# ssheybani/baby-vision-curriculum

Hardware: AMD Instinct MI355X
Metric: video clips/sec (node) VideoMAE-base 16x224^2 bf16 pretraining (higher is better)
Workload: dtype bf16; 1 GPU; VideoMAE-base (ViT-B/16 encoder, 4-layer decoder), 16x224x224 clips, tubelet 2, 90% tube mask, full training step (fwd + MSE + bwd + GradScaler + SGD-Nesterov); clips_per_gpu=256, global_batch=256, parallelism=dp1, weights=random init N(0,0.02), seed 0

## Files before the change

baby-vision-curriculum_amd/csrc/gemm8.hip:

```cpp
#include <stdio.h>
#include <stdlib.h>

#include <type_traits>

#include "gemm_tile.h"
#include "rowops.h"

namespace bvc {

namespace {

typedef __attribute__((ext_vector_type(4))) unsigned int u32x4;

#ifndef BVC_G8_ST_AUX
#define BVC_G8_ST_AUX 0
#endif
#ifndef BVC_G8_ROW_ST_AUX
#define BVC_G8_ROW_ST_AUX 0
#endif
constexpr uint32_t kInvalidBase = 0x80000000u;

struct Unit {
    int pi, m0, n0, kt0, nkt, split, tile;
};

__device__ __forceinline__ bf16x8 tr_frag(uint32_t region, uint32_t lane_base, uint32_t lane_swz, uint32_t chunk16, int ks) {
    const uint32_t a = region + lane_base + (chunk16 ^ lane_swz) + (uint32_t)ks * 8192u;
    bf16x4 lo = __builtin_amdgcn_ds_read_tr16_b64_v4i16((AS3 bf16x4*)(size_t)a);
    bf16x4 hi = __builtin_amdgcn_ds_read_tr16_b64_v4i16((AS3 bf16x4*)(size_t)(a + 1024u));
    return __builtin_shufflevector(lo, hi, 0, 1, 2, 3, 4, 5, 6, 7);
}

__device__ __forceinline__ float row16_sum(float v) {
    v += __builtin_bit_cast(float, __builtin_amdgcn_update_dpp(0, __builtin_bit_cast(int, v), 0x128, 0xF, 0xF, false));
    v += __builtin_bit_cast(float, __builtin_amdgcn_update_dpp(0, __builtin_bit_cast(int, v), 0x124, 0xF, 0xF, false));
    v += __builtin_bit_cast(float, __builtin_amdgcn_update_dpp(0, __builtin_bit_cast(int, v), 0x122, 0xF, 0xF, false));
    v += __builtin_bit_cast(float, __builtin_amdgcn_update_dpp(0, __builtin_bit_cast(int, v), 0x121, 0xF, 0xF, false));
    return v;
}

template <int BM, int BN>
__device__ __forceinline__ void decode_unit(const GemmGroup& g, int uid, Unit& u) {
    const bool tail = g.bal_units > 0 && uid >= g.bal_units;
    const int S = tail ? g.prob[0].split_k : 1;
    const int key = tail ? (uid - g.bal_units) * S : uid;
    int pi = 0;
#pragma unroll
    for (int i = 1; i < kMaxGroup; ++i)
        if (i < g.nprob && key >= g.tile_start[i]) pi = i;
    const GemmProblem& p = g.prob[pi];
    const int lid = tail ? (key - g.tile_start[pi]) / S : uid - g.tile_start[pi];
    const int tiles_n = (p.N + BN - 1) / BN, tiles_m = (p.M + BM - 1) / BM;
    const int ntiles = tiles_m * tiles_n;
    const int G = g.panel[pi];
    int split, tm, tn;
    if (tail) {
        split = S;
        tm = lid / tiles_n; tn = lid - tm * tiles_n;
    } else if (G > 0) {
        split = lid / ntiles;
        tile_of(lid - split * ntiles, tiles_m, tiles_n, G, tm, tn);
    } else if (G == -1) {
        split = lid / ntiles;
        const int w = lid - split * ntiles;
        if (tiles_n > tiles_m) { tm = w % tiles_m; tn = w / tiles_m; } else { tm = w / tiles_n; tn = w % tiles_n; }
    } else {
        split = lid % p.split_k;
        const int tl = lid / p.split_k;
        const bool m_fast = tiles_n > tiles_m;
        tm = m_fast ? tl % tiles_m : tl / tiles_n;
        tn = m_fast ? tl / tiles_m : tl % tiles_n;
    }
    const int nt_all = (p.K + 63) / 64;
    int per = (nt_all + p.split_k - 1) / p.split_k;
    per = (per + 1) & ~1;
    int kt0 = split * per;
    if (g.bal_units > 0) {
        kt0 = split * g.bal_lb;
        per = tail ? (nt_all - kt0 + 1) & ~1 : g.bal_lb;
    }
    u.pi = pi;
    u.m0 = __builtin_amdgcn_readfirstlane(tm * BM);
    u.n0 = __builtin_amdgcn_readfirstlane(tn * BN);
    u.kt0 = __builtin_amdgcn_readfirstlane(kt0);
    u.nkt = __builtin_amdgcn_readfirstlane(per);
    u.split = __builtin_amdgcn_readfirstlane(split);
    u.tile = __builtin_amdgcn_readfirstlane(tm * tiles_n + tn);
}

}

template <int BM, int BN, bool AT, bool BT, int EC>
__global__ __launch_bounds__(512, 1) void gemm8_kernel(const GemmGroup g, const int total_units) {
    extern __shared__ __attribute__((aligned(16))) char smem[];
    static_assert(BM == 256 || (BM == 128 && BN == 384), "128-row tiles: the 128 x 384 geometry only");
    static_assert(BN == 256 || BN == 128 || (BN == 384 && BM == 128), "column tiles of 256 / 128, or 384 with 128 rows");
    static_assert((EC == 4 || EC == 5) == (BM == 128 && !AT), "row epilogues (EC 4 / 5) are the k-contiguous-A instantiations of the 128 x 384 tile, and only they");
    static_assert(BM == 256 || EC == 4 || EC == 5 || (AT && BT && (EC == 2 || EC == 6)), "128 x 384 with transposed A: weight gradients");
    static_assert(EC != 6 || (AT && BT), "EC 6 (deterministic weight gradients) is a TN product");
    static_assert(EC != 4 || !BT, "EC 4 (residual + LayerNorm forward) is an NT product");
    constexpr int A_BYTES = BM * 64 * 2, B_BYTES = BN * 64 * 2, TILE = A_BYTES + B_BYTES;
    constexpr int WMR = BM / 2;
    constexpr int WN = BN / 4, TN = WN / 16, TM = WMR / 16, TMH = TM / 2;
    constexpr int NB = BN / 64, NBH = BN / 128, NAH = BM / 128;
    constexpr int n0c = AT ? NBH : (NB == 6 ? 3 : NB < 2 ? NB : 2), n1c = AT ? NAH : NB - n0c, n2c = AT ? NBH : BM / 128, n3c = AT ? NAH : BM / 128;
    constexpr int RT = BM / 128;
    constexpr int KMAX = (n0c > 2 || n1c > 2 || n2c > 2 || n3c > 2) ? 3 : 2;
    constexpr int PT = n0c + n1c + n2c + n3c;
#ifdef BVC_G8_DMA_LATE
    constexpr bool LATE = true;
#else
    constexpr bool LATE = false;
#endif
    constexpr int PAR_BYTES = EC == 4 ? 3 * BN * 4 : EC == 5 ? BN * 4 : 0, STAT_OFF = PAR_BYTES, COL_OFF = STAT_OFF + 4096;
    constexpr int CPR = BN == 384 ? 8 : WN / 8;
    constexpr int NSIDE = TM * (16 / (64 / CPR));
    static_assert(PT + 2 * NSIDE < 64, "vmcnt is a 6-bit counter");
    constexpr int WP = AT ? PT : n3c + n0c + n1c;
    constexpr int W1 = LATE ? n0c + n1c + n2c : PT;
    constexpr int W3 = LATE ? (AT ? n2c + n3c + n0c : n3c + n0c) : WP;

    const int tid = threadIdx.x, lane = tid & 63;
    const int wave = __builtin_amdgcn_readfirstlane(tid >> 6);
    const int wm = wave >> 2, wn = wave & 3;

    const int xcd = blockIdx.x & 7, slot_id = blockIdx.x >> 3, nslots = gridDim.x >> 3;
    const int xq = total_units >> 3, xr = total_units & 7;
    const int x_lo = xcd < xr ? xcd * (xq + 1) : xr * (xq + 1) + (xcd - xr) * xq;
    const int x_hi = x_lo + xq + (xcd < xr ? 1 : 0);
    int uid = x_lo + slot_id, u_step = nslots, u_hi = x_hi;
    if (EC == 2 && g.bal_units > 0) {
        u_step = 1;
        if (uid < x_hi) {
            u_hi = uid + 1;
        } else {
            const int J = xcd * nslots - x_lo + (uid - x_hi), I = 8 * nslots - g.bal_units;
            uid = g.bal_units + (J * g.bal_tiles) / I;
            u_hi = g.bal_units + ((J + 1) * g.bal_tiles) / I;
        }
    }
    if (uid >= u_hi) {
        if constexpr (EC == 5) {
            float* pr = g.prob[0].ln_part + (size_t)blockIdx.x * 2 * BN;
            for (int i = tid; i < 2 * BN; i += 512) pr[i] = 0.f;
        }
        return;
    }
    if constexpr (EC == 4 || EC == 5) {
        const int cnt = x_hi - x_lo, r = cnt % nslots, nmax = (cnt + nslots - 1) / nslots;
        int num = 0, den = 1;
        if (r > 0 && slot_id >= r) { num = slot_id - r + 1; den = nslots - r + 1; }
        else if (r == 0 && nmax >= 4) { num = slot_id; den = 2 * nslots; }
        const int quanta = __builtin_amdgcn_readfirstlane((int)((long long)g.stagger * num / den));
        for (int i = 0; i < quanta / 127; ++i) __builtin_amdgcn_s_sleep(127);
    }
    if (BVC_DBG(g, 1024) && (slot_id & 1)) {
        for (int i = 0; i < ((g.dbg >> 12) & 63); ++i) __builtin_amdgcn_s_sleep(127);
    }

    Unit su;
    decode_unit<BM, BN>(g, uid, su);
    int s_uid = uid, s_kt = 0;
    bool s_valid = true;
    __amdgpu_buffer_rsrc_t s_ra, s_rb;
    uint32_t s_la, s_lb, s_baseA, s_baseB, s_strideA, s_strideB;
    auto s_problem = [&]() {
        const GemmProblem& p = g.prob[su.pi];
        s_ra = make_rsrc(p.A, p.a_bytes);
        s_rb = make_rsrc(p.B, p.b_bytes);
        if constexpr (!AT) {
            const int r = 8 * wave + (lane >> 3);
            s_la = (uint32_t)((r * p.lda + (((lane & 7) ^ swz_rows(r)) << 3)) * 2);
            s_strideA = (uint32_t)(64 * p.lda * 2);
        } else {
            const int kr = 4 * wave + (lane >> 4);
            s_la = (uint32_t)((kr * p.lda + (((lane & 15) ^ swz_tr<128>(kr)) << 3)) * 2);
            s_strideA = (uint32_t)(32 * p.lda * 2);
        }
        if constexpr (!BT) {
            const int r = 8 * wave + (lane >> 3);
            s_lb = (uint32_t)((r * p.ldb + (((lane & 7) ^ swz_rows(r)) << 3)) * 2);
            s_strideB = (uint32_t)(64 * p.ldb * 2);
        } else {
            const int kr = 4 * wave + (lane >> 4);
            s_lb = (uint32_t)((kr * p.ldb + (((lane & 15) ^ swz_tr<128>(kr)) << 3)) * 2);
            s_strideB = (uint32_t)(32 * p.ldb * 2);
        }
    };
    auto s_ktile = [&]() {
        const GemmProblem& p = g.prob[su.pi];
        const int kt = su.kt0 + s_kt;
        const bool ok = s_valid && kt * 64 < p.K;
        const int k0 = kt * 64;
        s_baseA = !ok ? kInvalidBase : AT ? (uint32_t)((k0 * p.lda + su.m0) * 2) : (uint32_t)((su.m0 * p.lda + k0) * 2);
        s_baseB = !ok ? kInvalidBase : BT ? (uint32_t)((k0 * p.ldb + su.n0) * 2) : (uint32_t)((su.n0 * p.ldb + k0) * 2);
    };
    auto s_advance = [&]() {
        if (++s_kt == su.nkt) {
            s_kt = 0;
            s_uid += u_step;
            if (s_uid < u_hi) {
                const int old = su.pi;
                decode_unit<BM, BN>(g, s_uid, su);
                if (su.pi != old) s_problem();
            } else {
                s_valid = false;
            }
        }
        s_ktile();
    };
    const uint32_t lds_base = (uint32_t)(size_t)((AS3 char*)smem);
    const uint32_t lds0 = lds_base + (uint32_t)wave * 1024u;
    const uint32_t tr_base = (uint32_t)((8 * (lane >> 4) + ((lane >> 2) & 3)) * 256 + ((lane & 3) >> 1) * 16 + (lane & 1) * 8);
    const uint32_t tr_swz = (uint32_t)swz_tr<128>(8 * (lane >> 4) + ((lane >> 2) & 3)) << 4;
    auto b_region = [&](int j) -> uint32_t { return (uint32_t)(A_BYTES + ((wn * WN + 16 * j) >> 7) * 16384); };
    auto b_chunk16 = [&](int j) -> uint32_t { return (uint32_t)(2 * ((wn * WN + 16 * j) & 127)); };
    const uint32_t a_region = BM == 256 ? (uint32_t)wm * 16384u : 0u;
    const uint32_t a_chunk0 = BM == 256 ? 0u : (uint32_t)wm * 128u;
    auto load_a = [&](char* region, int j) {
        const uint32_t off = s_la + s_baseA + (AT ? (uint32_t)(j & 1) * s_strideA + (uint32_t)(j >> 1) * 256u : (uint32_t)j * s_strideA);
        glds16(s_ra, off, lds0 + (uint32_t)(region - smem) + (uint32_t)j * 8192u);
    };
    auto load_b = [&](char* region, int j) {
        const uint32_t off = s_lb + s_baseB + (BT ? (uint32_t)(j & 1) * s_strideB + (uint32_t)(j >> 1) * 256u : (uint32_t)j * s_strideB);
        glds16(s_rb, off, lds0 + (uint32_t)(region - smem) + (uint32_t)j * 8192u);
    };
    using I0 = std::integral_constant<int, 0>;
    using I1 = std::integral_constant<int, 1>;
    using I2 = std::integral_constant<int, 2>;
    using I3 = std::integral_constant<int, 3>;
    auto stage_one = [&](auto gi_, auto k_, char* buf) {
        constexpr int GI = decltype(gi_)::value, K = decltype(k_)::value;
        char* ra_ = buf;
        char* rb_ = buf + A_BYTES;
        if constexpr (!AT) {
            if constexpr (GI == 0) { if constexpr (K < n0c) load_b(rb_, K); }
            else if constexpr (GI == 1) { if constexpr (K < n1c) load_b(rb_, n0c + K); }
            else if constexpr (GI == 2) { if constexpr (K < n2c) load_a(ra_, BM == 256 ? (K == 0 ? 0 : 2) : 0); }
            else { if constexpr (K < n3c) load_a(ra_, BM == 256 ? (K == 0 ? 1 : 3) : 1); }
        } else {
            if constexpr (GI == 0) { if constexpr (K < NBH) load_b(rb_, 2 * K); }
            else if constexpr (GI == 1) { if constexpr (K < NAH) load_a(ra_, 2 * K); }
            else if constexpr (GI == 2) { if constexpr (K < NBH) load_b(rb_, 2 * K + 1); }
            else { if constexpr (K < NAH) load_a(ra_, 2 * K + 1); }
        }
        if constexpr (GI == 3 && K == KMAX - 1) s_advance();
    };
    auto stage_group = [&](auto gi_, char* buf) {
        stage_one(gi_, I0{}, buf); stage_one(gi_, I1{}, buf);
        if constexpr (KMAX == 3) stage_one(gi_, I2{}, buf);
    };
    auto stage_phase = [&](auto q_, auto k_, char* cur, char* oth) {
        constexpr int Q = decltype(q_)::value;
        if constexpr (Q == 0) stage_one(I2{}, k_, oth);
        else if constexpr (Q == 1) stage_one(I3{}, k_, oth);
        else if constexpr (Q == 2) stage_one(I0{}, k_, cur);
        else stage_one(I1{}, k_, cur);
    };

    char* const buf0 = smem;
    char* const buf1 = smem + TILE;
    constexpr int PARK = BN == 384 ? 16 * 48 * 4 : 16 * WN * 4;
    AS3 char* const wl = (AS3 char*)smem + 2 * TILE + wave * PARK;

    if constexpr (EC == 0) {
        const GemmProblem& p0 = g.prob[0];
        AS3 float* lbias = (AS3 float*)((AS3 char*)smem + 2 * TILE);
        const int npad = ((p0.N + BN - 1) / BN) * BN;
        for (int i = tid; i < npad; i += 512) lbias[i] = (p0.bias && i < p0.N) ? p0.bias[i] : 0.f;
        __syncthreads();
    }
    if constexpr (EC == 4 || EC == 5) {
        const GemmProblem& p0 = g.prob[0];
        AS3 float* lpar = (AS3 float*)((AS3 char*)smem + 2 * TILE);
        for (int i = tid; i < BN; i += 512) {
            if constexpr (EC == 4) {
                lpar[i] = p0.bias ? p0.bias[i] : 0.f;
                lpar[BN + i] = p0.ln_gamma[i];
                lpar[2 * BN + i] = p0.ln_beta[i];
            } else {
                lpar[i] = p0.ln_gamma[i];
            }
        }
        if constexpr (EC == 5) {
            AS3 float* lcol = (AS3 float*)((AS3 char*)smem + 2 * TILE + COL_OFF);
            for (int i = tid; i < 8 * 2 * WN; i += 512) lcol[i] = 0.f;
        }
        __syncthreads();
    }
    s_problem();
    s_ktile();
    stage_group(I0{}, buf0); stage_group(I1{}, buf0); stage_group(I2{}, buf0); stage_group(I3{}, buf0);
    stage_group(I0{}, buf1); stage_group(I1{}, buf1);
    wait_vmcnt<WP>();
    asm volatile("s_barrier" ::: "memory");
#ifndef BVC_G8_NO_STAGGER
    if (wm == 1) asm volatile("s_barrier" ::: "memory");
#endif

    Unit cu;
    decode_unit<BM, BN>(g, uid, cu);
    int after_epi = 0;


    while (true) {
        const GemmProblem& p = g.prob[cu.pi];
        f32x4 acc[TM][TN];
#pragma unroll
        for (int i = 0; i < TM; ++i)
#pragma unroll
            for (int j = 0; j < TN; ++j) acc[i][j] = f32x4{0.f, 0.f, 0.f, 0.f};
        float rsum[2] = {0.f, 0.f};
        const bool do_rowsum = (EC == 2 || EC == 6) && p.rowsum != nullptr && cu.n0 == 0;

        auto ktile = [&](auto rs_, char* cur, char* oth) {
            constexpr bool RS = decltype(rs_)::value;
            const char* la = cur;
            const char* lb = cur + A_BYTES;
            if constexpr (!AT) {
                bf16x8 bfr[2][TN];
                auto phase = [&](auto q_) {
                    constexpr int q = decltype(q_)::value;
                    __builtin_amdgcn_sched_barrier(0);
#ifdef BVC_G8_DMA_FIRST
                    if constexpr (!LATE) { stage_phase(q_, I0{}, cur, oth); stage_phase(q_, I1{}, cur, oth); if constexpr (KMAX == 3) stage_phase(q_, I2{}, cur, oth); }
#endif
                    uint32_t sw = tr_swz;
                    if constexpr (BT && q == 0) asm volatile("" : "+v"(sw));
                    if constexpr (q == 0) {
#pragma unroll
                        for (int ks = 0; ks < 2; ++ks)
#pragma unroll
                            for (int j = 0; j < TN; ++j)
                                bfr[ks][j] = BT ? tr_frag(lds_base + (uint32_t)(cur - smem) + b_region(j), tr_base, sw, b_chunk16(j), ks)
                                                : read_frag<BN, false>(lb, wn * WN + 16 * j, ks, lane);
                    }
                    bf16x8 af[2][RT];
#pragma unroll
                    for (int ks = 0; ks < 2; ++ks)
#pragma unroll
                        for (int ii = 0; ii < RT; ++ii)
                            af[ks][ii] = read_frag<256, false>(la, BM == 256 ? wm * WMR + 16 * (2 * q + ii) : 32 * q + 16 * wm, ks, lane);
#ifndef BVC_G8_DMA_FIRST
                    if constexpr (!LATE) { stage_phase(q_, I0{}, cur, oth); stage_phase(q_, I1{}, cur, oth); if constexpr (KMAX == 3) stage_phase(q_, I2{}, cur, oth); }
#endif
                    if constexpr (q == 1) {
                        if (after_epi == 0) wait_vmcnt<W1>();
                        else if (after_epi == NSIDE) wait_vmcnt<W1 + NSIDE>();
                        else if (after_epi == 2 * NSIDE) wait_vmcnt<W1 + 2 * NSIDE>();
                    }
                    if constexpr (q == 3) wait_vmcnt<W3>();
                    asm volatile("s_barrier" ::: "memory");
                    __builtin_amdgcn_sched_barrier(0);
                    __builtin_amdgcn_s_setprio(1);
                    constexpr int NM = 2 * RT * TN;
#pragma unroll
                    for (int t = 0; t < NM; ++t) {
                        const int ks = t / (RT * TN), ii = (t / TN) % RT, j = t % TN;
                        acc[RT * q + ii][j] = __builtin_amdgcn_mfma_f32_16x16x32_bf16(bfr[ks][j], af[ks][ii], acc[RT * q + ii][j], 0, 0, 0);
                        if constexpr (LATE) {
                            if (t == NM / 4 - 1) stage_phase(q_, I0{}, cur, oth);
                            if (t == NM / 2 - 1) stage_phase(q_, I1{}, cur, oth);
                        }
                    }
                    __builtin_amdgcn_s_setprio(0);
                    __builtin_amdgcn_sched_barrier(0);
                    asm volatile("s_barrier" ::: "memory");
                };
                phase(I0{}); phase(I1{}); phase(I2{}); phase(I3{});
            } else {
                bf16x8 bfr[TN];
                auto phase = [&](auto q_) {
                    constexpr int q = decltype(q_)::value;
                    constexpr int ks = q >> 1, mh = q & 1;
                    __builtin_amdgcn_sched_barrier(0);
                    bf16x8 af[TMH];
                    uint32_t sw = tr_swz;
                    asm volatile("" : "+v"(sw));
                    const uint32_t slot = lds_base + (uint32_t)(cur - smem);
                    if constexpr (mh == 0) {
#pragma unroll
                        for (int j = 0; j < TN; ++j) bfr[j] = tr_frag(slot + b_region(j), tr_base, sw, b_chunk16(j), ks);
                    }
#pragma unroll
                    for (int ii = 0; ii < TMH; ++ii) af[ii] = tr_frag(slot + a_region, tr_base, sw, a_chunk0 + 32u * (TMH * mh + ii), ks);
                    if constexpr (!LATE) {
                        stage_phase(q_, I0{}, cur, oth); stage_phase(q_, I1{}, cur, oth);
                        if constexpr (KMAX == 3) stage_phase(q_, I2{}, cur, oth);
                    }
                    if constexpr (q == 1) {
                        if (after_epi == 0) wait_vmcnt<W1>();
                        else if (after_epi == NSIDE) wait_vmcnt<W1 + NSIDE>();
                        else if (after_epi == 2 * NSIDE) wait_vmcnt<W1 + 2 * NSIDE>();
                    }
                    if constexpr (q == 3) wait_vmcnt<W3>();
                    asm volatile("s_barrier" ::: "memory");
                    __builtin_amdgcn_sched_barrier(0);
                    __builtin_amdgcn_s_setprio(1);
                    constexpr int NM = TMH * TN;
#pragma unroll
                    for (int t = 0; t < NM; ++t) {
                        const int ii = t / TN, j = t % TN;
                        acc[TMH * mh + ii][j] = __builtin_amdgcn_mfma_f32_16x16x32_bf16(bfr[j], af[ii], acc[TMH * mh + ii][j], 0, 0, 0);
                        if constexpr (LATE) {
                            if (t == NM / 4 - 1) stage_phase(q_, I0{}, cur, oth);
                            if (t == NM / 2 - 1) stage_phase(q_, I1{}, cur, oth);
                        }
                    }
                    if (RS && do_rowsum && wn < TMH) {
                        bf16x8 a;
                        if constexpr (TMH == 4) {
                            switch (wn) {
                                case 0: a = af[0]; break;
                                case 1: a = af[1]; break;
                                case 2: a = af[2]; break;
                                default: a = af[3]; break;
                            }
                        } else {
                            a = wn == 0 ? af[0] : af[1];
                        }
                        union { bf16x8 v; uint32_t u[4]; } w;
                        w.v = a;
                        float t0 = 0.f, t1 = 0.f;
#pragma unroll
                        for (int e = 0; e < 4; ++e) {
                            t0 += __uint_as_float(w.u[e] << 16);
                            t1 += __uint_as_float(w.u[e] & 0xffff0000u);
                        }
                        rsum[mh] += t0 + t1;
                    }
                    __builtin_amdgcn_s_setprio(0);
                    __builtin_amdgcn_sched_barrier(0);
                    asm volatile("s_barrier" ::: "memory");
                };
                phase(I0{}); phase(I1{}); phase(I2{}); phase(I3{});
            }
            after_epi = 0;
        };

        for (int kt = 0; kt < cu.nkt; kt += 2) {
            ktile(std::bool_constant<EC == 2 || EC == 6>{}, buf0, buf1);
            ktile(std::bool_constant<EC == 2 || EC == 6>{}, buf1, buf0);
        }

        const int m0 = cu.m0, n0 = cu.n0;
        const int epi = p.epi, Mrows = p.M, Ncols = p.N, ldc = p.ldc;
        int seg_shift = 0;
        if constexpr (EC == 4 || EC == 5) {
            if (p.seg_rows > 0) {
                const int upc = p.seg_rows >> 7, u = m0 >> 7, c = u / upc;
                seg_shift = __builtin_amdgcn_readfirstlane(c * p.seg_stride + p.seg_off + ((u - c * upc) << 7) - m0);
            }
        }
        const float alpha = p.alpha_dev ? p.alpha * p.alpha_dev[0] : p.alpha;
        constexpr int UNITS = WN / 4;
        constexpr int RPU = 64 / CPR;
        constexpr int U = 16 / RPU;
        static_assert(NSIDE == TM * U, "epilogue geometry");
        int nstores = 0;
        constexpr uint32_t kDrop = 0xFFFFFFF0u;
        auto park = [&](int i) {
            const int row = lane & 15;
#pragma unroll
            for (int j = 0; j < TN; ++j) {
                const int unit = (4 * j + (lane >> 4)) ^ (row & (UNITS - 1));
                *reinterpret_cast<AS3 f32x4*>(wl + row * (WN * 4) + unit * 16) = acc[i][j];
            }
        };
        const bool atomic = p.split_k > 1 || g.accum != 0;
        if constexpr (EC == 0) {
            const __amdgpu_buffer_rsrc_t rc = make_rsrc(p.C, BVC_DBG(g, 1) ? 0u : kDrop);
            const __amdgpu_buffer_rsrc_t rc2 = make_rsrc(p.C2 ? p.C2 : p.C, BVC_DBG(g, 1) ? 0u : kDrop);
            const AS3 float* lbias = (const AS3 float*)((AS3 char*)smem + 2 * TILE);
            const int q4 = lane >> 4;
            f32x4 bj[TN];
#pragma unroll
            for (int j = 0; j < TN; ++j) {
                const int nb = n0 + wn * WN + 16 * j + 4 * q4;
                bj[j] = *reinterpret_cast<const AS3 f32x4*>(lbias + nb);
            }
            const bool two_out = epi == EPI_GELU;
            const bool relu = epi == EPI_RELU;
            const int ncol = n0 + wn * WN + 16 * (q4 & 1) + 8 * (q4 >> 1);
#pragma unroll
            for (int i = 0; i < TM; ++i) {
                const int m = m0 + wm * WMR + 16 * i + (lane & 15);
#pragma unroll
                for (int jp = 0; jp < TN / 2; ++jp) {
                    float va[4], vb[4];
#pragma unroll
                    for (int e = 0; e < 4; ++e) {
                        va[e] = acc[i][2 * jp][e] * alpha + bj[2 * jp][e];
                        vb[e] = acc[i][2 * jp + 1][e] * alpha + bj[2 * jp + 1][e];
                    }
                    if (relu) {
#pragma unroll
                        for (int e = 0; e < 4; ++e) { va[e] = fmaxf(va[e], 0.f); vb[e] = fmaxf(vb[e], 0.f); }
                    }
                    const int n = ncol + 32 * jp;
                    const uint32_t o = (m < Mrows && n < Ncols) ? (uint32_t)(((size_t)m * ldc + n) * 2) : kDrop;
                    auto emit = [&](__amdgpu_buffer_rsrc_t r) {
                        uint32_t a0 = pack2bf(va[0], va[1]), a1 = pack2bf(va[2], va[3]);
                        uint32_t b0 = pack2bf(vb[0], vb[1]), b1 = pack2bf(vb[2], vb[3]);
                        const auto s0 = __builtin_amdgcn_permlane16_swap(a0, b0, false, false);
                        const auto s1 = __builtin_amdgcn_permlane16_swap(a1, b1, false, false);
                        __builtin_amdgcn_raw_buffer_store_b128(u32x4{s0[0], s1[0], s0[1], s1[1]}, r, o, 0, BVC_G8_ST_AUX);
                    };
                    if (two_out) {
                        float vv[8], gg[8];
#pragma unroll
                        for (int e = 0; e < 4; ++e) { vv[e] = va[e]; vv[4 + e] = vb[e]; }
                        gelu_split(vv, gg);
#pragma unroll
                        for (int e = 0; e < 4; ++e) { va[e] = vv[e]; vb[e] = vv[4 + e]; }
                        emit(rc);
#pragma unroll
                        for (int e = 0; e < 4; ++e) { va[e] = gg[e]; vb[e] = gg[4 + e]; }
                        emit(rc2);
                    } else {
                        emit(rc);
                    }
                }
            }
            nstores = two_out ? 2 * NSIDE : NSIDE;
        } else if constexpr (EC == 4) {
            const uint32_t ext = (uint32_t)Mrows * (uint32_t)(BN * 4);
            const __amdgpu_buffer_rsrc_t rres = make_rsrc(p.resid + (size_t)seg_shift * BN, ext), rc = make_rsrc(p.C, ext), rc2 = make_rsrc(p.C2, ext / 2);
            const __amdgpu_buffer_rsrc_t rmu = make_rsrc(p.ln_mean, (uint32_t)Mrows * 4u), rrs = make_rsrc(p.ln_rstd, (uint32_t)Mrows * 4u);
            const AS3 float* lpar = (const AS3 float*)((AS3 char*)smem + 2 * TILE);
            AS3 float* lstat = (AS3 float*)((AS3 char*)smem + 2 * TILE + STAT_OFF);
            const int q4 = lane >> 4, r16 = lane & 15;
            const int cw = wn * WN + 4 * q4;
            const float eps = p.ln_eps;
            const uint32_t obase = (uint32_t)(m0 + 16 * wm + r16) * (uint32_t)(BN * 4) + (uint32_t)cw * 4u;
            f32x4 rs[2][TN];
            auto issue = [&](auto i_) {
                constexpr int i = decltype(i_)::value;
#pragma unroll
                for (int j = 0; j < TN; ++j)
                    rs[i & 1][j] = __builtin_bit_cast(f32x4, __builtin_amdgcn_raw_buffer_load_b128(rres, obase + (uint32_t)(i * 32 * BN * 4 + 64 * j), 0, 0));
            };
            auto tile = [&](auto i_) {
                constexpr int i = decltype(i_)::value;
                __builtin_amdgcn_sched_barrier(0);
                if constexpr (i + 1 < TM) issue(std::integral_constant<int, i + 1>{});
                __builtin_amdgcn_sched_barrier(0);
                float sum = 0.f;
#pragma unroll
                for (int j = 0; j < TN; ++j) {
                    const f32x4 bj = *reinterpret_cast<const AS3 f32x4*>(lpar + cw + 16 * j);
                    acc[i][j] = (acc[i][j] * alpha + bj) + rs[i & 1][j];
                    __builtin_amdgcn_raw_buffer_store_b128(__builtin_bit_cast(u32x4, acc[i][j]), rc, obase + (uint32_t)(i * 32 * BN * 4 + 64 * j), 0, BVC_G8_ROW_ST_AUX);
                    sum += (acc[i][j][0] + acc[i][j][1]) + (acc[i][j][2] + acc[i][j][3]);
                }
                sum += __shfl_xor(sum, 16, 64);
                sum += __shfl_xor(sum, 32, 64);
                const float mw = sum * (1.f / WN);
                float sq = 0.f;
#pragma unroll
                for (int j = 0; j < TN; ++j)
#pragma unroll
                    for (int e = 0; e < 4; ++e) { const float d = acc[i][j][e] - mw; sq += d * d; }
                sq += __shfl_xor(sq, 16, 64);
                sq += __shfl_xor(sq, 32, 64);
                if (q4 == 0) *reinterpret_cast<AS3 f32x2*>(lstat + ((wm * 64 + 16 * i + r16) * 4 + wn) * 2) = f32x2{sum, sq};
            };
            issue(I0{});
            wait_vmcnt<0>();
#pragma unroll
            for (int j = 0; j < TN; ++j) asm volatile("" : "+v"(rs[0][j]));
            tile(I0{}); tile(I1{}); tile(I2{}); tile(I3{});
            asm volatile("s_waitcnt lgkmcnt(0)\n\ts_barrier" ::: "memory");
#pragma unroll
            for (int i = 0; i < TM; ++i) {
                asm volatile("" ::: "memory");
                const AS3 f32x4* sp = reinterpret_cast<const AS3 f32x4*>(lstat + (wm * 64 + 16 * i + r16) * 8);
                const f32x4 a = sp[0], b = sp[1];
                const float mean = ((a[0] + a[2]) + (b[0] + b[2])) * (1.f / BN);
                const float d0 = a[0] * (1.f / WN) - mean, d1 = a[2] * (1.f / WN) - mean, d2 = b[0] * (1.f / WN) - mean, d3 = b[2] * (1.f / WN) - mean;
                const float m2 = ((a[1] + a[3]) + (b[1] + b[3])) + (float)WN * ((d0 * d0 + d1 * d1) + (d2 * d2 + d3 * d3));
                const float rstd = rsqrtf(m2 * (1.f / BN) + eps);
                const int m = m0 + 32 * i + 16 * wm + r16;
                if (wn == 0 && q4 == 0) {
                    __builtin_amdgcn_raw_buffer_store_b32(__float_as_uint(mean), rmu, (uint32_t)m * 4u, 0, 0);
                    __builtin_amdgcn_raw_buffer_store_b32(__float_as_uint(rstd), rrs, (uint32_t)m * 4u, 0, 0);
                }
                const uint32_t o2 = ((uint32_t)m * (uint32_t)BN + (uint32_t)(wn * WN + 16 * (q4 & 1) + 8 * (q4 >> 1))) * 2u;
#pragma unroll
                for (int jp = 0; jp < TN / 2; ++jp) {
                    const f32x4 ga = *reinterpret_cast<const AS3 f32x4*>(lpar + BN + cw + 32 * jp), gb = *reinterpret_cast<const AS3 f32x4*>(lpar + BN + cw + 32 * jp + 16);
                    const f32x4 ba = *reinterpret_cast<const AS3 f32x4*>(lpar + 2 * BN + cw + 32 * jp), bb = *reinterpret_cast<const AS3 f32x4*>(lpar + 2 * BN + cw + 32 * jp + 16);
                    const f32x4 ya = ((acc[i][2 * jp] - mean) * rstd) * ga + ba;
                    const f32x4 yb = ((acc[i][2 * jp + 1] - mean) * rstd) * gb + bb;
                    const uint32_t a0 = pack2bf(ya[0], ya[1]), a1 = pack2bf(ya[2], ya[3]), b0 = pack2bf(yb[0], yb[1]), b1 = pack2bf(yb[2], yb[3]);
                    const auto s0 = __builtin_amdgcn_permlane16_swap(a0, b0, false, false);
                    const auto s1 = __builtin_amdgcn_permlane16_swap(a1, b1, false, false);
                    __builtin_amdgcn_raw_buffer_store_b128(u32x4{s0[0], s1[0], s0[1], s1[1]}, rc2, o2 + 64u * jp, 0, BVC_G8_ROW_ST_AUX);
                }
            }
        } else if constexpr (EC == 5) {
            const uint32_t ext = (uint32_t)Mrows * (uint32_t)(BN * 4);
            const __amdgpu_buffer_rsrc_t rx = make_rsrc(p.ln_x, ext), rd = make_rsrc(reinterpret_cast<float*>(p.C) + (size_t)seg_shift * BN, ext), rc2 = make_rsrc(p.C2, ext / 2);
            const __amdgpu_buffer_rsrc_t rmu = make_rsrc(p.ln_mean, (uint32_t)Mrows * 4u), rrs = make_rsrc(p.ln_rstd, (uint32_t)Mrows * 4u);
            const AS3 float* lpar = (const AS3 float*)((AS3 char*)smem + 2 * TILE);
            AS3 float* lstat = (AS3 float*)((AS3 char*)smem + 2 * TILE + STAT_OFF);
            AS3 float* lcol = (AS3 float*)((AS3 char*)smem + 2 * TILE + COL_OFF) + wave * 2 * WN;
            const int q4 = lane >> 4, r16 = lane & 15;
            const int cw = wn * WN + 4 * q4;
            const int mrow = m0 + 16 * wm + r16;
            const uint32_t obase = (uint32_t)mrow * (uint32_t)(BN * 4) + (uint32_t)cw * 4u;
            const uint32_t o2base = ((uint32_t)mrow * (uint32_t)BN + (uint32_t)(wn * WN + 16 * (q4 & 1) + 8 * (q4 >> 1))) * 2u;
            f32x4 xr[2][TN], dr[TN];
            float mu[2], rsd[2];
            auto issue = [&](auto i_) {
                constexpr int i = decltype(i_)::value;
                mu[i & 1] = __uint_as_float(__builtin_amdgcn_raw_buffer_load_b32(rmu, (uint32_t)(mrow + 32 * i) * 4u, 0, 0));
                rsd[i & 1] = __uint_as_float(__builtin_amdgcn_raw_buffer_load_b32(rrs, (uint32_t)(mrow + 32 * i) * 4u, 0, 0));
#pragma unroll
                for (int j = 0; j < TN; ++j)
                    xr[i & 1][j] = __builtin_bit_cast(f32x4, __builtin_amdgcn_raw_buffer_load_b128(rx, obase + (uint32_t)(i * 32 * BN * 4 + 64 * j), 0, 0));
            };
            auto tile = [&](auto i_) {
                constexpr int i = decltype(i_)::value, b = i & 1;
                __builtin_amdgcn_sched_barrier(0);
#pragma unroll
                for (int j = 0; j < TN; ++j)
                    dr[j] = __builtin_bit_cast(f32x4, __builtin_amdgcn_raw_buffer_load_b128(rd, obase + (uint32_t)(i * 32 * BN * 4 + 64 * j), 0, 0));
                if constexpr (i + 1 < TM) issue(std::integral_constant<int, i + 1>{});
                __builtin_amdgcn_sched_barrier(0);
                float s1 = 0.f, s2 = 0.f;
#pragma unroll
                for (int j = 0; j < TN; ++j) {
                    const f32x4 gam = *reinterpret_cast<const AS3 f32x4*>(lpar + cw + 16 * j);
                    const f32x4 gv = acc[i][j] * alpha;
                    const f32x4 xh = (xr[b][j] - mu[b]) * rsd[b];
                    const f32x4 gg = gv * gam;
                    f32x4 tg = gv * xh, tb = gv;
                    s1 += (gg[0] + gg[1]) + (gg[2] + gg[3]);
                    const f32x4 gx = gg * xh;
                    s2 += (gx[0] + gx[1]) + (gx[2] + gx[3]);
                    xr[b][j] = xh;
                    acc[i][j] = gg;
#pragma unroll
                    for (int e = 0; e < 4; ++e) {
                        tg[e] = row16_sum(tg[e]);
                        tb[e] = row16_sum(tb[e]);
                    }
                    if (r16 == 0) {
                        AS3 f32x4* cg = reinterpret_cast<AS3 f32x4*>(lcol + 16 * j + 4 * q4);
                        AS3 f32x4* cb = reinterpret_cast<AS3 f32x4*>(lcol + WN + 16 * j + 4 * q4);
                        *cg = *cg + tg;
                        *cb = *cb + tb;
                    }
                }
                s1 += __shfl_xor(s1, 16, 64);
                s1 += __shfl_xor(s1, 32, 64);
                s2 += __shfl_xor(s2, 16, 64);
                s2 += __shfl_xor(s2, 32, 64);
                if (q4 == 0) *reinterpret_cast<AS3 f32x2*>(lstat + ((wm * 64 + 16 * i + r16) * 4 + wn) * 2) = f32x2{s1, s2};
                asm volatile("s_waitcnt lgkmcnt(0)\n\ts_barrier" ::: "memory");
                const AS3 f32x4* sp = reinterpret_cast<const AS3 f32x4*>(lstat + (wm * 64 + 16 * i + r16) * 8);
                const f32x4 sa = sp[0], sb = sp[1];
                const float c1 = ((sa[0] + sa[2]) + (sb[0] + sb[2])) * (1.f / BN), c2 = ((sa[1] + sa[3]) + (sb[1] + sb[3])) * (1.f / BN);
#pragma unroll
                for (int j = 0; j < TN; ++j) {
                    acc[i][j] = ((acc[i][j] - c1) - xr[b][j] * c2) * rsd[b] + dr[j];
                    __builtin_amdgcn_raw_buffer_store_b128(__builtin_bit_cast(u32x4, acc[i][j]), rd, obase + (uint32_t)(i * 32 * BN * 4 + 64 * j), 0, BVC_G8_ROW_ST_AUX);
                }
#pragma unroll
                for (int jp = 0; jp < TN / 2; ++jp) {
                    const f32x4 ya = acc[i][2 * jp], yb = acc[i][2 * jp + 1];
                    const uint32_t a0 = pack2bf(ya[0], ya[1]), a1 = pack2bf(ya[2], ya[3]), b0 = pack2bf(yb[0], yb[1]), b1 = pack2bf(yb[2], yb[3]);
                    const auto w0 = __builtin_amdgcn_permlane16_swap(a0, b0, false, false);
                    const auto w1 = __builtin_amdgcn_permlane16_swap(a1, b1, false, false);
                    __builtin_amdgcn_raw_buffer_store_b128(u32x4{w0[0], w1[0], w0[1], w1[1]}, rc2, o2base + (uint32_t)(i * 32 * BN * 2 + 64 * jp), 0, BVC_G8_ROW_ST_AUX);
                }
            };
            issue(I0{});
            wait_vmcnt<0>();
            asm volatile("" : "+v"(mu[0]), "+v"(rsd[0]));
#pragma unroll
            for (int j = 0; j < TN; ++j) asm volatile("" : "+v"(xr[0][j]));
            tile(I0{}); tile(I1{}); tile(I2{}); tile(I3{});
        } else if constexpr (BN == 384) {
            const __amdgpu_buffer_rsrc_t rca = make_rsrc(p.C, kDrop);
            const __amdgpu_buffer_rsrc_t rsl = make_rsrc(EC == 6 && atomic ? p.partial + (size_t)cu.split * Mrows * Ncols : p.C, kDrop);
#pragma unroll
            for (int i = 0; i < TM; ++i) {
#pragma unroll
                for (int ps = 0; ps < 2; ++ps) {
                    const int prow = lane & 15;
#pragma unroll
                    for (int jj = 0; jj < 3; ++jj)
                        *reinterpret_cast<AS3 f32x4*>(wl + prow * 192 + (4 * jj + (lane >> 4)) * 16) = acc[i][3 * ps + jj];
#pragma unroll
                    for (int t = 0; t < 16 * 48 / 64; ++t) {
                        const int idx = t * 64 + lane;
                        const int row = idx / 48, col = idx % 48;
                        const int m = m0 + wm * WMR + 16 * i + row, n = n0 + wn * WN + 48 * ps + col;
                        const float v = *reinterpret_cast<const AS3 float*>(wl + row * 192 + col * 4) * alpha;
                        const uint32_t o = (m < Mrows && n < Ncols) ? (uint32_t)(((size_t)m * ldc + n) * 4) : kDrop;
                        if constexpr (EC == 6) {
                            if (atomic) __builtin_amdgcn_raw_buffer_store_b32(__float_as_uint(v), rsl, (m < Mrows && n < Ncols) ? (uint32_t)(((size_t)m * Ncols + n) * 4) : kDrop, 0, 0);
                            else __builtin_amdgcn_raw_buffer_store_b32(__float_as_uint(v), rca, o, 0, 0);
                        } else {
                            if (atomic) __builtin_amdgcn_raw_ptr_buffer_atomic_fadd_f32(v, rca, o, 0, 0);
                            else __builtin_amdgcn_raw_buffer_store_b32(__float_as_uint(v), rca, o, 0, 0);
                        }
                    }
                }
            }
        } else if ((EC == 2 || EC == 6) && atomic) {
            const __amdgpu_buffer_rsrc_t rca = make_rsrc(EC == 6 ? p.partial + (size_t)cu.split * Mrows * Ncols : p.C, kDrop);
#pragma unroll
            for (int i = 0; i < TM; ++i) {
                park(i);
#pragma unroll
                for (int t = 0; t < 16 * WN / 64; ++t) {
                    const int idx = t * 64 + lane;
                    const int row = idx / WN, col = idx % WN;
                    const int m = m0 + wm * WMR + 16 * i + row, n = n0 + wn * WN + col;
                    const int unit = (col >> 2) ^ (row & (UNITS - 1));
                    const float v = *reinterpret_cast<const AS3 float*>(wl + row * (WN * 4) + unit * 16 + (col & 3) * 4) * alpha;
                    const uint32_t o = (m < Mrows && n < Ncols) ? (uint32_t)(((size_t)m * (EC == 6 ? Ncols : ldc) + n) * 4) : kDrop;
                    if constexpr (EC == 6) __builtin_amdgcn_raw_buffer_store_b32(__float_as_uint(v), rca, o, 0, 0);
                    else __builtin_amdgcn_raw_ptr_buffer_atomic_fadd_f32(v, rca, o, 0, 0);
                }
            }
        } else {
            const int cc = lane % CPR;
            const int n = n0 + wn * WN + cc * 8;
            const bool ncol_ok = n < Ncols;
            const __amdgpu_buffer_rsrc_t rc = make_rsrc(p.C, kDrop);
            const __amdgpu_buffer_rsrc_t rc2 = make_rsrc((EC == 0 || EC == 1) && p.C2 ? p.C2 : p.C, kDrop);
            const bool have_c2 = p.C2 != nullptr;
            auto offs = [&](int m, int ld, int esz) -> uint32_t {
                return (m < Mrows && ncol_ok) ? (uint32_t)(((size_t)m * ld + n) * esz) : kDrop;
            };
            f32x4 bias0 = {0.f, 0.f, 0.f, 0.f}, bias1 = {0.f, 0.f, 0.f, 0.f};
            if constexpr (EC != 2 && EC != 6) {
                const __amdgpu_buffer_rsrc_t rbias = make_rsrc(p.bias, p.bias ? kDrop : 0u);
                const uint32_t ob = ncol_ok ? (uint32_t)n * 4u : kDrop;
                bias0 = __builtin_bit_cast(f32x4, __builtin_amdgcn_raw_buffer_load_b128(rbias, ob, 0, 0));
                bias1 = __builtin_bit_cast(f32x4, __builtin_amdgcn_raw_buffer_load_b128(rbias, ob, 16, 0));
            }
// ... 286 lines not shown
```

Before: 3364 clips/s.

## Replace XOR swizzle with sub-tiled LDS layout for transposed weight-gradient GEMM tiles

For the 128-row TN (weight-gradient) GEMM instantiations, the k-major LDS staging layout changes from an XOR-swizzled layout to a sub-tiled arrangement. Global-to-LDS source offsets and the ds_read_tr lane addresses are recomputed to match. Per-slot base addresses are precomputed once, so the inner loop reads fragments with constant offsets instead of recomputing XORed addresses every phase. The aim is fewer address VALU ops and bank conflicts in the MFMA loop, at the cost of more live VGPRs and possibly less coalesced global loads.

After: 3381 clips/s, median of 6. No clear change (+0.5%).

```diff
diff --git a/baby-vision-curriculum_amd/csrc/gemm8.hip b/baby-vision-curriculum_amd/csrc/gemm8.hip
--- a/baby-vision-curriculum_amd/csrc/gemm8.hip
+++ b/baby-vision-curriculum_amd/csrc/gemm8.hip
@@ -24,11 +24,35 @@
     int pi, m0, n0, kt0, nkt, split, tile;
 };
 
-__device__ __forceinline__ bf16x8 tr_frag(uint32_t region, uint32_t lane_base, uint32_t lane_swz, uint32_t chunk16, int ks) {
-    const uint32_t a = region + lane_base + (chunk16 ^ lane_swz) + (uint32_t)ks * 8192u;
-    bf16x4 lo = __builtin_amdgcn_ds_read_tr16_b64_v4i16((AS3 bf16x4*)(size_t)a);
-    bf16x4 hi = __builtin_amdgcn_ds_read_tr16_b64_v4i16((AS3 bf16x4*)(size_t)(a + 1024u));
+#ifdef BVC_G8_TR_XOR
+constexpr bool kTrXor = true;
+#else
+constexpr bool kTrXor = false;
+#endif
+template <bool SUB>
+__device__ __forceinline__ uint32_t tr_lane_base(int lane) {
+    const int g = lane >> 4, q = (lane >> 2) & 3, p = lane & 3;
+    if constexpr (!SUB) return (uint32_t)((8 * g + q) * 256 + (p >> 1) * 16 + (p & 1) * 8);
+    else return (uint32_t)(((g >> 1) << 12) | ((g & 1) << 7) | (q << 5) | (p << 3));
+}
+template <bool SUB>
+__device__ __forceinline__ void tr_src(int wave, int lane, int& kr, int& chunk) {
+    if constexpr (!SUB) {
+        kr = 4 * wave + (lane >> 4);
+        chunk = (lane & 15) ^ swz_tr<128>(kr);
+    } else {
+        kr = ((wave >> 2) << 4) | (((lane >> 3) & 1) << 3) | (((wave >> 1) & 1) << 2) | ((lane >> 1) & 3);
+        chunk = ((((wave & 1) << 2) | (lane >> 4)) << 1) | (lane & 1);
+    }
+}
+template <bool SUB>
+__device__ __forceinline__ bf16x8 tr_frag(uint32_t addr, uint32_t off) {
+    bf16x4 lo = __builtin_amdgcn_ds_read_tr16_b64_v4i16((AS3 bf16x4*)(size_t)(addr + off));
+    bf16x4 hi = __builtin_amdgcn_ds_read_tr16_b64_v4i16((AS3 bf16x4*)(size_t)(addr + off + (SUB ? 2048u : 1024u)));
     return __builtin_shufflevector(lo, hi, 0, 1, 2, 3, 4, 5, 6, 7);
+}
+__device__ __forceinline__ bf16x8 tr_frag_xor(uint32_t region, uint32_t lane_base, uint32_t lane_swz, uint32_t chunk16, int ks) {
+    return tr_frag<false>(region + lane_base + (chunk16 ^ lane_swz) + (uint32_t)ks * 8192u, 0u);
 }
 
 __device__ __forceinline__ float row16_sum(float v) {
@@ -112,6 +136,7 @@
 #else
     constexpr bool LATE = false;
 #endif
+    constexpr bool SUB = !kTrXor && AT && BT && BM == 128;
     constexpr int PAR_BYTES = EC == 4 ? 3 * BN * 4 : EC == 5 ? BN * 4 : 0, STAT_OFF = PAR_BYTES, COL_OFF = STAT_OFF + 4096;
     constexpr int CPR = BN == 384 ? 8 : WN / 8;
     constexpr int NSIDE = TM * (16 / (64 / CPR));
@@ -173,8 +198,9 @@
             s_la = (uint32_t)((r * p.lda + (((lane & 7) ^ swz_rows(r)) << 3)) * 2);
             s_strideA = (uint32_t)(64 * p.lda * 2);
         } else {
-            const int kr = 4 * wave + (lane >> 4);
-            s_la = (uint32_t)((kr * p.lda + (((lane & 15) ^ swz_tr<128>(kr)) << 3)) * 2);
+            int kr, c;
+            tr_src<SUB>(wave, lane, kr, c);
+            s_la = (uint32_t)((kr * p.lda + (c << 3)) * 2);
             s_strideA = (uint32_t)(32 * p.lda * 2);
         }
         if constexpr (!BT) {
@@ -182,8 +208,9 @@
             s_lb = (uint32_t)((r * p.ldb + (((lane & 7) ^ swz_rows(r)) << 3)) * 2);
             s_strideB = (uint32_t)(64 * p.ldb * 2);
         } else {
-            const int kr = 4 * wave + (lane >> 4);
-            s_lb = (uint32_t)((kr * p.ldb + (((lane & 15) ^ swz_tr<128>(kr)) << 3)) * 2);
+            int kr, c;
+            tr_src<SUB>(wave, lane, kr, c);
+            s_lb = (uint32_t)((kr * p.ldb + (c << 3)) * 2);
             s_strideB = (uint32_t)(32 * p.ldb * 2);
         }
     };
@@ -211,12 +238,37 @@
     };
     const uint32_t lds_base = (uint32_t)(size_t)((AS3 char*)smem);
     const uint32_t lds0 = lds_base + (uint32_t)wave * 1024u;
-    const uint32_t tr_base = (uint32_t)((8 * (lane >> 4) + ((lane >> 2) & 3)) * 256 + ((lane & 3) >> 1) * 16 + (lane & 1) * 8);
+    const uint32_t tr_base = tr_lane_base<SUB>(lane);
     const uint32_t tr_swz = (uint32_t)swz_tr<128>(8 * (lane >> 4) + ((lane >> 2) & 3)) << 4;
     auto b_region = [&](int j) -> uint32_t { return (uint32_t)(A_BYTES + ((wn * WN + 16 * j) >> 7) * 16384); };
     auto b_chunk16 = [&](int j) -> uint32_t { return (uint32_t)(2 * ((wn * WN + 16 * j) & 127)); };
     const uint32_t a_region = BM == 256 ? (uint32_t)wm * 16384u : 0u;
     const uint32_t a_chunk0 = BM == 256 ? 0u : (uint32_t)wm * 128u;
+    constexpr int NTB = BN == 384 ? TN / 2 : 1;
+    uint32_t tr_a[2] = {0u, 0u}, tr_b[2][NTB] = {};
+    if constexpr (SUB) {
+#pragma unroll
+        for (int s = 0; s < 2; ++s) {
+            const uint32_t slot = lds_base + (uint32_t)(s * TILE) + tr_base;
+            if constexpr (AT) {
+                tr_a[s] = slot + (BM == 256 ? (uint32_t)wm * 16384u : (uint32_t)wm * 1024u);
+                asm volatile("" : "+v"(tr_a[s]));
+            }
+            if constexpr (BT) {
+#pragma unroll
+                for (int jj = 0; jj < NTB; ++jj) {
+                    const int c = wn * WN + 32 * jj;
+                    tr_b[s][jj] = slot + (uint32_t)(A_BYTES + (c >> 7) * 16384 + ((c >> 4) & 7) * 256);
+                    asm volatile("" : "+v"(tr_b[s][jj]));
+                }
+            }
+        }
+    }
+    auto b_frag = [&](int s, int j, int ks) -> bf16x8 {
+        if constexpr (BN == 384) return tr_frag<SUB>(tr_b[s][j >> 1], (uint32_t)((j & 1) * 256 + ks * 8192));
+        else return tr_frag<SUB>(tr_b[s][0], (uint32_t)(j * 256 + ks * 8192));
+    };
+    auto a_frag = [&](int s, int t, int ks) -> bf16x8 { return tr_frag<SUB>(tr_a[s], (uint32_t)(t * 256 + ks * 8192)); };
     auto load_a = [&](char* region, int j) {
         const uint32_t off = s_la + s_baseA + (AT ? (uint32_t)(j & 1) * s_strideA + (uint32_t)(j >> 1) * 256u : (uint32_t)j * s_strideA);
         glds16(s_ra, off, lds0 + (uint32_t)(region - smem) + (uint32_t)j * 8192u);
@@ -313,8 +365,9 @@
         float rsum[2] = {0.f, 0.f};
         const bool do_rowsum = (EC == 2 || EC == 6) && p.rowsum != nullptr && cu.n0 == 0;
 
-        auto ktile = [&](auto rs_, char* cur, char* oth) {
+        auto ktile = [&](auto rs_, auto slot_, char* cur, char* oth) {
             constexpr bool RS = decltype(rs_)::value;
+            constexpr int SL = decltype(slot_)::value;
             const char* la = cur;
             const char* lb = cur + A_BYTES;
             if constexpr (!AT) {
@@ -326,14 +379,16 @@
                     if constexpr (!LATE) { stage_phase(q_, I0{}, cur, oth); stage_phase(q_, I1{}, cur, oth); if constexpr (KMAX == 3) stage_phase(q_, I2{}, cur, oth); }
 #endif
                     uint32_t sw = tr_swz;
-                    if constexpr (BT && q == 0) asm volatile("" : "+v"(sw));
+                    if constexpr (!SUB && BT && q == 0) asm volatile("" : "+v"(sw));
                     if constexpr (q == 0) {
 #pragma unroll
                         for (int ks = 0; ks < 2; ++ks)
 #pragma unroll
-                            for (int j = 0; j < TN; ++j)
-                                bfr[ks][j] = BT ? tr_frag(lds_base + (uint32_t)(cur - smem) + b_region(j), tr_base, sw, b_chunk16(j), ks)
-                                                : read_frag<BN, false>(lb, wn * WN + 16 * j, ks, lane);
+                            for (int j = 0; j < TN; ++j) {
+                                if constexpr (!BT) bfr[ks][j] = read_frag<BN, false>(lb, wn * WN + 16 * j, ks, lane);
+                                else if constexpr (!SUB) bfr[ks][j] = tr_frag_xor(lds_base + (uint32_t)(cur - smem) + b_region(j), tr_base, sw, b_chunk16(j), ks);
+                                else bfr[ks][j] = b_frag(SL, j, ks);
+                            }
                     }
                     bf16x8 af[2][RT];
 #pragma unroll
@@ -375,15 +430,24 @@
                     constexpr int ks = q >> 1, mh = q & 1;
                     __builtin_amdgcn_sched_barrier(0);
                     bf16x8 af[TMH];
-                    uint32_t sw = tr_swz;
-                    asm volatile("" : "+v"(sw));
-                    const uint32_t slot = lds_base + (uint32_t)(cur - smem);
-                    if constexpr (mh == 0) {
-#pragma unroll
-                        for (int j = 0; j < TN; ++j) bfr[j] = tr_frag(slot + b_region(j), tr_base, sw, b_chunk16(j), ks);
-                    }
-#pragma unroll
-                    for (int ii = 0; ii < TMH; ++ii) af[ii] = tr_frag(slot + a_region, tr_base, sw, a_chunk0 + 32u * (TMH * mh + ii), ks);
+                    if constexpr (!SUB) {
+                        uint32_t sw = tr_swz;
+                        asm volatile("" : "+v"(sw));
+                        const uint32_t slot = lds_base + (uint32_t)(cur - smem);
+                        if constexpr (mh == 0) {
+#pragma unroll
+                            for (int j = 0; j < TN; ++j) bfr[j] = tr_frag_xor(slot + b_region(j), tr_base, sw, b_chunk16(j), ks);
+                        }
+#pragma unroll
+                        for (int ii = 0; ii < TMH; ++ii) af[ii] = tr_frag_xor(slot + a_region, tr_base, sw, a_chunk0 + 32u * (TMH * mh + ii), ks);
+                    } else {
+                        if constexpr (mh == 0) {
+#pragma unroll
+                            for (int j = 0; j < TN; ++j) bfr[j] = b_frag(SL, j, ks);
+                        }
+#pragma unroll
+                        for (int ii = 0; ii < TMH; ++ii) af[ii] = a_frag(SL, TMH * mh + ii, ks);
+                    }
                     if constexpr (!LATE) {
                         stage_phase(q_, I0{}, cur, oth); stage_phase(q_, I1{}, cur, oth);
                         if constexpr (KMAX == 3) stage_phase(q_, I2{}, cur, oth);
@@ -439,8 +503,8 @@
         };
 
         for (int kt = 0; kt < cu.nkt; kt += 2) {
-            ktile(std::bool_constant<EC == 2 || EC == 6>{}, buf0, buf1);
-            ktile(std::bool_constant<EC == 2 || EC == 6>{}, buf1, buf0);
+            ktile(std::bool_constant<EC == 2 || EC == 6>{}, I0{}, buf0, buf1);
+            ktile(std::bool_constant<EC == 2 || EC == 6>{}, I1{}, buf1, buf0);
         }
 
         const int m0 = cu.m0, n0 = cu.n0;
```
